# lock042/siril

Measured on AMD Instinct MI355X. Metric: Mpix/s stacked (100x6000x4000 fp32 sigma-clip) at 1/2/4/8 MI355X; % HBM roofline, higher is better.
Workload: dtype f32

## Files before the change

include/sirilgpu.h:

```cpp
#ifndef SIRILGPU_H
#define SIRILGPU_H

#include <stddef.h>
#include <stdint.h>

#ifdef __cplusplus
extern "C" {
#endif

#define SGPU_OK               0
#define SGPU_GENERIC_ERROR   (-1)
#define SGPU_SEQUENCE_ERROR  (-2)
#define SGPU_CANCEL          (-9)
#define SGPU_ALLOC_ERROR     (-10)
#define SGPU_NO_DEVICE       (-20)
#define SGPU_BAD_ARGUMENT    (-21)

enum sgpu_rejection {
	SGPU_NO_REJEC = 0, SGPU_PERCENTILE = 1, SGPU_SIGMA = 2, SGPU_MAD = 3,
	SGPU_SIGMEDIAN = 4, SGPU_WINSORIZED = 5, SGPU_LINEARFIT = 6, SGPU_GESDT = 7
};
enum sgpu_normalization {
	SGPU_NO_NORM = 0, SGPU_ADDITIVE = 1, SGPU_MULTIPLICATIVE = 2,
	SGPU_ADDITIVE_SCALING = 3, SGPU_MULTIPLICATIVE_SCALING = 4
// ... 66 lines not shown
		long *start_row, long *block_height, int *channel, int *nb_blocks, long *largest);
void sgpu_feather_mask_size(long width, long height, long *mask_width, long *mask_height);
int sgpu_feather_masks_device(sgpu_context *ctx, const void *d_frames, int elem_size, int nframes,
		long width, long height, long frame_stride, float *d_masks);
int sgpu_feather_block_area(long width, long height, long start_row, long block_height, int shifty,
		int registered, int *plane_row, int *area_h, int *mask_row, int *mask_h);
int sgpu_feather_block_device(sgpu_context *ctx, const float *d_masks, int nframes, long width,
		long height, long start_row, long block_height, const int *shifty, const int *placex,
		long canvas_width, float feather, int fits_order, float *d_planes, long plane_stride);

int sgpu_set_input_bitpix(sgpu_context *ctx, int bitpix);

long sgpu_last_exact_pixels(sgpu_context *ctx);

int sgpu_last_wz_deferred(sgpu_context *ctx, long long out[2]);

long sgpu_last_order_sensitive(sgpu_context *ctx, int *idx, long cap);

int sgpu_set_exact_only(sgpu_context *ctx, int on);


typedef struct sgpu_multi sgpu_multi;
int sgpu_multi_init(const int *devices, int ndevices, sgpu_multi **multi);
void sgpu_multi_release(sgpu_multi *multi);
int sgpu_multi_size(const sgpu_multi *multi);
sgpu_context *sgpu_multi_context(sgpu_multi *multi, int index);
int sgpu_multi_stack_rows(sgpu_multi *multi, const float *frames, int nframes, long width, long rows,
		long frame_stride, const sgpu_stack_params *params, float *out, uint16_t *rej_lo,
		uint16_t *rej_hi, uint64_t counts[2]);
int sgpu_multi_stack_rows_u16(sgpu_multi *multi, const uint16_t *frames16, int nframes, long width,
// ... 347 lines not shown
```

siril_amd/_lib.py:

```python
from __future__ import annotations

import ctypes as C
import os

PKG = os.path.dirname(os.path.abspath(__file__))
LIB_PATH = os.environ.get("SGPU_LIB") or os.path.join(PKG, "libsirilgpu.so")

EXPORTS = (
    "sgpu_abi_version", "sgpu_device_count", "sgpu_init", "sgpu_release", "sgpu_set_stream", "sgpu_synchronize",
    "sgpu_last_error", "sgpu_stack_rows", "sgpu_stack_rows_device", "sgpu_last_exact_pixels", "sgpu_last_order_sensitive",
    "sgpu_last_wz_deferred", "sgpu_set_exact_only", "sgpu_set_timing", "sgpu_last_timing", "sgpu_stack_rows_u16",
    "sgpu_stack_rows_u16_device", "sgpu_dft_shifts", "sgpu_dft_register_device",
    "sgpu_quality_estimate_device", "sgpu_quality_estimate", "sgpu_normalize_quality",
    "sgpu_quality_estimate_u16_device", "sgpu_quality_estimate_u16",
    "sgpu_fft_richardson_lucy", "sgpu_naive_richardson_lucy", "sgpu_rl_fft", "sgpu_rl_naive",
    "sgpu_rl_fft_device", "sgpu_rl_naive_device", "sgpu_rl_set_memory", "sgpu_rl_last_conv_launches",
    "sgpu_rl_last_iter_flops", "sgpu_dft_shifts_cfa", "sgpu_dft_register_cfa_device",
    "sgpu_interpolate_nongreen_device", "sgpu_debayer_buffer_new_float",
    "sgpu_debayer_buffer_superpixel_float", "sgpu_debayer_device", "sgpu_superpixel_device", "sgpu_free",
    "sgpu_debayer_buffer_new_ushort", "sgpu_debayer_u16_device",
    "sgpu_bgnoise_device", "sgpu_bgnoise_u16_device", "sgpu_bgnoise", "sgpu_bgnoise_u16",
    "sgpu_stack_seq", "sgpu_stack_seq_ex", "sgpu_norm_stats_device", "sgpu_norm_stats",
    "sgpu_norm_stats_u16_device", "sgpu_norm_stats_u16", "sgpu_norm_factors",
    "sgpu_fits_info", "sgpu_fits_read_rows", "sgpu_fits_read_rows_ex", "sgpu_fits_write",
    "sgpu_norm_to_0_1_range_device", "sgpu_multi_init", "sgpu_multi_release", "sgpu_multi_size",
    "sgpu_multi_context", "sgpu_multi_stack_rows", "sgpu_multi_stack_rows_u16", "sgpu_row_bands",
# ... 122 lines not shown
        L.sgpu_stack_rows_planes.argtypes = [vp, vp, vp, vp] + list(L.sgpu_stack_rows.argtypes[2:])
        L.sgpu_stack_rows_planes_device.restype = C.c_int
        L.sgpu_stack_rows_planes_device.argtypes = [vp, vp, vp, vp] + list(L.sgpu_stack_rows_device.argtypes[2:])
        L.sgpu_stack_rows_u16_device.restype = C.c_int
        L.sgpu_stack_rows_u16_device.argtypes = [vp, vp, C.c_int, C.c_long, C.c_long, C.c_long,
                                                 C.POINTER(StackParams), vp, vp, vp, vp, vp]
        L.sgpu_stack_rows_u16_planes_device.restype = C.c_int
        L.sgpu_stack_rows_u16_planes_device.argtypes = [vp, vp, vp, vp] + list(L.sgpu_stack_rows_u16_device.argtypes[2:])
        L.sgpu_dft_shifts.restype = C.c_int
        L.sgpu_dft_shifts.argtypes = [vp, vp, vp, C.c_int, C.c_int, vp, vp]
        L.sgpu_dft_register_device.restype = C.c_int
        L.sgpu_dft_register_device.argtypes = [vp, vp, C.c_long, vp, C.c_long, C.c_long, C.c_int,
                                               C.c_int, vp, vp]
        L.sgpu_last_exact_pixels.restype = C.c_long
        L.sgpu_last_exact_pixels.argtypes = [vp]
        L.sgpu_last_wz_deferred.restype = C.c_int
        L.sgpu_last_wz_deferred.argtypes = [vp, vp]
        L.sgpu_last_order_sensitive.restype = C.c_long
        L.sgpu_last_order_sensitive.argtypes = [vp, vp, C.c_long]
        L.sgpu_set_exact_only.restype = C.c_int
        L.sgpu_set_exact_only.argtypes = [vp, C.c_int]
        L.sgpu_set_input_bitpix.restype = C.c_int
        L.sgpu_set_input_bitpix.argtypes = [vp, C.c_int]
        L.sgpu_set_timing.restype = C.c_int
        L.sgpu_set_timing.argtypes = [vp, C.c_int]
        L.sgpu_last_timing.restype = C.c_int
        L.sgpu_last_timing.argtypes = [vp, C.POINTER(C.c_float)]
        u, i, f = C.c_uint, C.c_int, C.c_float
        for name in ("sgpu_fft_richardson_lucy", "sgpu_naive_richardson_lucy"):
            getattr(L, name).restype = i
# ... 231 lines not shown
```

siril_amd/csrc/sgpu_capi.cpp:

```cpp
#include <hip/hip_runtime.h>

#include <algorithm>
#include <cmath>
#include <cstdio>
#include <cstdlib>
#include <cstring>
#include <string>
#include <thread>
#include <vector>

#include "../../include/sirilgpu.h"
#include "sgpu_internal.h"
#include "sgpu_kparams.h"

namespace sgpu {
int launch_sorted_16(const KParams &, hipStream_t);
int launch_sorted_32(const KParams &, hipStream_t);
int launch_sorted_64(const KParams &, hipStream_t);
int launch_sorted_128(const KParams &, hipStream_t);
int launch_sorted_256(const KParams &, hipStream_t);
int launch_sorted_512(const KParams &, hipStream_t);
int launch_sorted_1024(const KParams &, hipStream_t);
int launch_sorted16_16(const KParams &, hipStream_t);
int launch_sorted16_32(const KParams &, hipStream_t);
// ... 243 lines not shown
    return n;
}

int sgpu_last_wz_deferred(sgpu_context *c, long long out[2]) {
    if (!c || !out) return fail(SGPU_BAD_ARGUMENT, "null argument");
    out[0] = out[1] = 0;
    HIP_TRY(hipStreamSynchronize(c->stream));
    if (!c->wz_cnt.p) return SGPU_OK;
    int t[2] = {0, 0};
    HIP_TRY(hipMemcpy(t, (int *)c->wz_cnt.p + sgpu::kWzDefOff, sizeof t, hipMemcpyDeviceToHost));
    out[0] = t[0];
    out[1] = t[1];
    return SGPU_OK;
}

long sgpu_last_order_sensitive(sgpu_context *c, int *idx, long cap) {
    if (!c) return fail(SGPU_BAD_ARGUMENT, "null context");
    if (hipStreamSynchronize(c->stream) != hipSuccess) return SGPU_NO_DEVICE;
    if (!c->last_mean || !c->fb2_count.p) return 0;
    int n = 0;
    if (hipMemcpy(&n, c->fb2_count.p, sizeof(int), hipMemcpyDeviceToHost) != hipSuccess) return SGPU_NO_DEVICE;
    if (idx && cap > 0 && n > 0 &&
        hipMemcpy(idx, c->fb2_list.p, (size_t)std::min<long>(cap, n) * sizeof(int), hipMemcpyDeviceToHost) !=
            hipSuccess)
        return SGPU_NO_DEVICE;
    return n;
}

}

// ... 133 lines not shown
        if (hipGetLastError() != hipSuccess) return fail(SGPU_NO_DEVICE, "count fold launch failed");
    }
    return SGPU_OK;
}

int run_launch_body(sgpu_context *c, KParams k, bool has_shift) {
    hipStream_t s = c->stream;
    const int N = k.nframes;
    int r;
    if ((r = c->fb_list.ensure(k.npix * sizeof(int))) || (r = c->fb_count.ensure(sizeof(int))))
        return r;
    k.fb_list = (int *)c->fb_list.p;
    k.fb_count = (int *)c->fb_count.p;
    HIP_TRY(hipMemsetAsync(k.fb_count, 0, sizeof(int), s));
    if (c->wz_cnt.p) HIP_TRY(hipMemsetAsync((int *)c->wz_cnt.p + 2 * sgpu::kWzMaxChunks, 0, 3 * sizeof(int), s));
    static const int wz_mode = std::getenv("SGPU_WZ") ? std::atoi(std::getenv("SGPU_WZ")) : 2;
    static const int wz_rw = std::getenv("SGPU_WZ_RW") ? std::atoi(std::getenv("SGPU_WZ_RW")) : 64;
    k.wz_mode = wz_mode;
    k.wz_rw = wz_rw;
    if (!k.frames16 && k.rtype == SGPU_NO_REJEC) {
        if ((r = c->fb2_list.ensure(k.npix * sizeof(int))) || (r = c->fb2_count.ensure(sizeof(int)))) return r;
        k.fb2_list = (int *)c->fb2_list.p;
        k.fb2_count = (int *)c->fb2_count.p;
        HIP_TRY(hipMemsetAsync(k.fb2_count, 0, sizeof(int), s));
    }
    c->last_mean = k.rtype == SGPU_NO_REJEC && !k.frames16;
    if (k.rtype == SGPU_WINSORIZED && wz_mode) {
        if ((r = c->fb2_list.ensure(k.npix * sizeof(int))) || (r = c->fb2_count.ensure(sizeof(int)))) return r;
        k.fb2_list = (int *)c->fb2_list.p;
        k.fb2_count = (int *)c->fb2_count.p;
        HIP_TRY(hipMemsetAsync(k.fb2_count, 0, sizeof(int), s));
        const int npw = sorted_capacity(N);
        const long long R = npw <= 128 ? 64 : npw / 2 + 16;
// ... 428 lines not shown
```

siril_amd/csrc/sgpu_kparams.h:

```cpp
#pragma once
#include <stdint.h>

namespace sgpu {

enum Rejection : int {
    NO_REJEC = 0, PERCENTILE = 1, SIGMA = 2, MAD = 3, SIGMEDIAN = 4,
    WINSORIZED = 5, LINEARFIT = 6, GESDT = 7,
    KMEDIAN = 16
};
enum Normalization : int {
    NO_NORM = 0, ADDITIVE = 1, MULTIPLICATIVE = 2, ADDITIVE_SCALING = 3,
    MULTIPLICATIVE_SCALING = 4
};

struct KParams {
    const float *frames;
    long long frame_stride;
    long long npix;
    int W;
    int nframes;
    int rtype;
    float sig0, sig1;
    int norm;
    const double *scale, *offset, *mul;
// ... 12 lines not shown
    int *fb_count;
    int *fb2_list;
    int *fb2_count;
    long long wz_pix0, wz_cnt;
    float *wz_ranks;
    double *wz_mom;
    int *wz_meta;
    void *wz_state;
    int *wz_list_in, *wz_list_out;
    int *wz_lcount;
    void *wz_ws;
    long long wz_ws_bytes;
    long long wz_chunk;
    int *wz_tcnt;
    int wz_mode;
    int wz_split;
    int *wz_scnt;
    int *wz_def;
    int wz_rw;
    float *scratch;
    long long scratch_threads;
    const uint16_t *frames16;
    uint16_t *out16;
    int out_f32;
    double out16_mul;
    unsigned long long *prof;
};

struct WzSplit {
    int cap;
// ... 17 lines not shown
```

siril_amd/csrc/stack_sorted_gw.h:

```cpp
#pragma once
#ifndef SGPU_GW16
#define SGPU_GW16 1, 4
#endif
#ifndef SGPU_GW16_LOOP
#define SGPU_GW16_LOOP 1, 4
#endif
#ifndef SGPU_GW32
#define SGPU_GW32 1, 4
#endif
#ifndef SGPU_GW32_LOOP
#define SGPU_GW32_LOOP 1, 4
#endif
#ifndef SGPU_GW64
#define SGPU_GW64 1, 3
#endif
#ifndef SGPU_GW64_LOOP
#define SGPU_GW64_LOOP 1, 3
#endif
#ifndef SGPU_GW128
#define SGPU_GW128 1, 2
#endif
#ifndef SGPU_GW128_LOOP
#define SGPU_GW128_LOOP 2, 4
#endif
// ... 18 lines not shown
#ifndef SGPU_WZ_PREP_G128
#define SGPU_WZ_PREP_G128 1
#endif
#ifndef SGPU_WZ_PREP_G128_XF
#define SGPU_WZ_PREP_G128_XF 1
#endif
#ifndef SGPU_WZ_PREP_W128
#define SGPU_WZ_PREP_W128 6
#endif
#ifndef SGPU_WZ_PREP_W128_G2
#define SGPU_WZ_PREP_W128_G2 4
#endif
#ifndef SGPU_WZ_PREP_W128_G1
#define SGPU_WZ_PREP_W128_G1 3
#endif
#ifndef SGPU_WZ_PREP4_RS0
#define SGPU_WZ_PREP4_RS0 20
#endif
#ifndef SGPU_WZ_PREP4_RSSTEP
#define SGPU_WZ_PREP4_RSSTEP 4
#endif
static_assert((SGPU_WZ_PREP_G128 == 1 || SGPU_WZ_PREP_G128 == 2 || SGPU_WZ_PREP_G128 == 4) &&
              (SGPU_WZ_PREP_G128_XF == 1 || SGPU_WZ_PREP_G128_XF == 2 || SGPU_WZ_PREP_G128_XF == 4),
              "prep kernel: 1, 2 or 4 lanes per pixel");
```

siril_amd/csrc/stack_sorted_inst.h:

```cpp
#pragma once
#include "stack_sorted_impl.h"
#include "stack_sorted_gw.h"
#include "stack_wz.h"
#ifndef SGPU_WZ_RRW
#define SGPU_WZ_RRW 4
#endif

#ifndef SGPU_WZ_TAIL_PASSES
#define SGPU_WZ_TAIL_PASSES 2
#endif
static_assert(SGPU_WZ_TAIL_PASSES >= 1 && SGPU_WZ_TAIL_PASSES <= 2,
              "each of the two stripe-counter sets is zeroed once per chunk and appended to by one pass");

#include <algorithm>
#include <cstdlib>
#include <type_traits>

#ifndef SGPU_WZ_MOMENTS
#define SGPU_WZ_MOMENTS 1
#endif
#ifndef SGPU_WZ_W128
#define SGPU_WZ_W128 4
#endif
#ifndef SGPU_WZ_W
// ... 27 lines not shown
        if (hipStreamCreateWithFlags(&a->s2, hipStreamNonBlocking) != hipSuccess) return -1;
        if (hipStreamCreateWithFlags(&a->s3, hipStreamNonBlocking) != hipSuccess) return -1;
        hipEvent_t *ev[6] = {&a->start, &a->prep[0], &a->prep[1], &a->rounds[0], &a->rounds[1], &a->tails};
        for (hipEvent_t *e : ev)
            if (hipEventCreateWithFlags(e, hipEventDisableTiming) != hipSuccess) return -1;
    }
    return 0;
}

using KernelFn = void (*)(KParams);
KernelFn rs_kernel_128(int kind, int xf, int rs);
KernelFn prep4_kernel_128(int xf, int rs);
int rs_pick_prep4(int N);
KernelFn prep1_kernel_128(int xf, int rs);
int rs_pick_prep1(int N);
KernelFn rs_kernel_256(int kind, int xf, int rs);
KernelFn rs_kernel_512(int kind, int xf, int rs);
template <int NP> inline KernelFn rs_kernel(int kind, int xf, int rs) {
    if constexpr (NP == 128) return rs_kernel_128(kind, xf, rs);
    else if constexpr (NP == 256) return rs_kernel_256(kind, xf, rs);
    else if constexpr (NP == 512) return rs_kernel_512(kind, xf, rs);
    else return nullptr;
}
inline bool launch_fn(KernelFn f, unsigned grid, unsigned block, hipStream_t s, const KParams &p) {
    KParams k = p;
    void *args[] = {&k};
    return hipLaunchKernel((const void *)f, dim3(grid), dim3(block), args, 0, s) == hipSuccess;
}

inline int wz_exact_block(int N) {
    const long long per = 24ll * N;
    int t = 64;
    while (t > 4 && (long long)t * per > 65536) t >>= 1;
    return (long long)t * per <= 65536 ? t : 0;
}

constexpr int kWzMinChunks = 1;
constexpr long long kWzMinChunkPix = 1LL << 19;

template <int NP, int G, int RT, int W, int U16 = 0>
static int launch_one(const KParams &p, hipStream_t s) {
    const long long threads = p.npix * (long long)G;
    const unsigned grid = (unsigned)((threads + 255) / 256);
    constexpr int E = NP / G;
    const int rs = rs_pick(E, G, p.nframes);
    const unsigned long long es = U16 ? 2ull : 4ull;
    if ((unsigned long long)(G - 1) * (unsigned long long)p.frame_stride * es +
            (unsigned long long)p.npix * es >= 0xffffffffull)
        return 1;
    constexpr bool WZM = SGPU_WZ_MOMENTS && RT == WINSORIZED && NP >= 128;
    if constexpr (WZM) if (!U16 || (p.wz_mode >= 2 && p.wz_mode <= 4 && p.wz_ws)) {
        auto two_kernel = [&](auto pg_tag) -> int {
            constexpr int PG = decltype(pg_tag)::value;
            const bool ovl = p.wz_mode == 3 || (p.wz_mode == 2 && NP <= 128);
            const int nbuf = ovl ? 2 : 1;
            constexpr int R = RankStore<NP, PG>::R;
            constexpr int PE = NP / PG;
            constexpr int PW = (NP == 128 && !U16) ? (PG == 4 ? SGPU_WZ_PREP_W128 : PG == 2 ? SGPU_WZ_PREP_W128_G2
                                                                                            : SGPU_WZ_PREP_W128_G1)
                                                   : W;
            (void)PW;
            const long long per = (long long)R * 4 + 3 * 8 + 16 + (long long)sizeof(WzState) + 8;
            const long long wsb = (p.wz_ws_bytes / nbuf) & ~4095LL;
            long long ch = std::min<long long>(p.npix, ((wsb - 4096) / per) & ~255LL);
            ch = std::min<long long>(ch, (1LL << 23) - 256);
            ch = std::min<long long>(ch, (0xffffffffLL / R) & ~255LL);
            ch = std::min<long long>(ch, ((1LL << 32) / (4LL * NP) - 256) & ~255LL);
            static const int minch = std::getenv("SGPU_WZ_MINCH") ? std::atoi(std::getenv("SGPU_WZ_MINCH")) : kWzMinChunks;
            if (ovl && minch > 1 && p.npix > (long long)minch * kWzMinChunkPix)
                ch = std::min<long long>(ch, ((p.npix + minch - 1) / minch + 255) & ~255LL);
            if (p.wz_chunk > 0) ch = std::min<long long>(ch, (p.wz_chunk + 255) & ~255LL);
            if (ch <= 0) return 1;
            WzAux *aux = nullptr;
            hipStream_t sp = s;
            if (ovl) {
                if (wz_aux(aux)) return -1;
                sp = aux->s2;
                if (hipEventRecord(aux->start, s) != hipSuccess || hipStreamWaitEvent(sp, aux->start, 0) != hipSuccess)
                    return -1;
            }
            KParams q = p;
            int *lists[2], *cnts = nullptr;
            const long long nch = (p.npix + ch - 1) / ch;
            const int et = wz_exact_block(p.nframes);
            const bool tails = !U16 && ovl && p.wz_tcnt && nch <= kWzMaxChunks && et > 0 && p.wz_rw != 100;
            auto place = [&](int b) {
                char *base = (char *)p.wz_ws + (long long)b * wsb;
                q.wz_ranks = (float *)base;
                q.wz_mom = (double *)(base + (((long long)R * 4 * ch + 255) & ~255LL));
                q.wz_meta = (int *)((char *)q.wz_mom + 3 * 8 * ch);
                q.wz_state = (void *)((char *)q.wz_meta + 16 * ch);
                lists[0] = (int *)((char *)q.wz_state + (long long)sizeof(WzState) * ch);
                lists[1] = lists[0] + ch;
                cnts = lists[1] + ch;
            };
            KernelFn prep_rs = nullptr;
            constexpr bool kOwnPrep = NP == 128 && !U16 && (PG == 4 || PG == 1);
            if constexpr (NP == 128 && !U16 && PG == 4) {
                prep_rs = prep4_kernel_128(p.shiftx ? 1 : 0, rs_pick_prep4(p.nframes));
                if (!prep_rs) return -1;
            } else if constexpr (NP == 128 && !U16 && PG == 1) {
                prep_rs = prep1_kernel_128(p.shiftx ? 1 : 0, rs_pick_prep1(p.nframes));
                if (!prep_rs) return -1;
            } else if constexpr (!U16 && PE == 64) {
                const int prs = rs_pick(PE, PG, p.nframes);
                if (prs < PE) prep_rs = rs_kernel<NP>(0, p.shiftx ? 1 : 0, prs);
            }
            int k = 0;
            for (long long p0 = 0; p0 < p.npix; p0 += ch, k++) {
                const int b = k % nbuf;
                place(b);
                q.wz_pix0 = p0;
                q.wz_cnt = std::min(ch, p.npix - p0);
                if (tails) {
                    q.fb2_list = p.fb2_list + p0;
                    q.fb2_count = p.wz_tcnt + 2 * k;
                    q.fb_list = p.fb_list + p0;
                    q.fb_count = p.wz_tcnt + 2 * k + 1;
                }
                const unsigned g1 = (unsigned)((q.wz_cnt * PG + 255) / 256), g2 = (unsigned)((q.wz_cnt + 255) / 256);
                if (ovl && k >= nbuf && hipStreamWaitEvent(sp, aux->rounds[b], 0) != hipSuccess) return -1;
                if (prep_rs) {
                    if (!launch_fn(prep_rs, g1, 256, sp, q)) return -1;
                } else if constexpr (kOwnPrep) {
                    return -1;
                } else if (p.shiftx) hipLaunchKernelGGL((k_stack_wz_prep<NP, PG, 1, PW, PE, U16>), g1, 256, 0, sp, q);
                else hipLaunchKernelGGL((k_stack_wz_prep<NP, PG, 0, PW, PE, U16>), g1, 256, 0, sp, q);
                if (ovl && (hipEventRecord(aux->prep[b], sp) != hipSuccess ||
                            hipStreamWaitEvent(s, aux->prep[b], 0) != hipSuccess))
                    return -1;
                if constexpr (U16 && NP <= 128) {
                    if (p.wz_rw == 64)
                        hipLaunchKernelGGL((k_stack_wz_rounds_lds<NP, 1, PG>), dim3((unsigned)((q.wz_cnt + 63) / 64)), 64, 0,
                                           s, q, WzSplit{});
                    else
                        hipLaunchKernelGGL((k_stack_wz_rounds<NP, 5, 1, PG>), g2, 256, 0, s, q);
                } else if constexpr (U16) {
// ... 15 lines not shown
                        case 6: hipLaunchKernelGGL((k_stack_wz_rounds<NP, 6, 0, PG>), g2, 256, 0, s, q); break;
                        case 64:
                            if constexpr (NP <= 128) {
                                const unsigned nblk = (unsigned)((q.wz_cnt + 63) / 64);
                                WzSplit sp{};
                                if (p.wz_split > 0 && p.wz_scnt) {
                                    sp.cap = p.wz_split;
                                    sp.bps = (int)((nblk + kWzStripes - 1) / kWzStripes);
                                    sp.nstripes = (int)((nblk + sp.bps - 1) / sp.bps);
                                    sp.list_out = lists[0];
                                    sp.cnt_out = p.wz_scnt;
                                    if (hipMemsetAsync(p.wz_scnt, 0, 2 * kWzStripes * kWzStripeStep * sizeof(int), s) !=
                                        hipSuccess)
                                        return -1;
                                }
                                hipLaunchKernelGGL((k_stack_wz_rounds_lds<NP, 0, PG>), dim3(nblk), 64, 0, s, q, sp);
                                for (int pass = 0; sp.cap && pass < SGPU_WZ_TAIL_PASSES; pass++) {
                                    sp.list_in = lists[pass & 1];
                                    sp.cnt_in = p.wz_scnt + (pass & 1) * kWzStripes * kWzStripeStep;
                                    sp.list_out = lists[(pass + 1) & 1];
                                    sp.cnt_out = p.wz_scnt + ((pass + 1) & 1) * kWzStripes * kWzStripeStep;
                                    sp.def = p.wz_def ? p.wz_def + pass : nullptr;
                                    hipLaunchKernelGGL((k_stack_wz_tail<NP, PG>), dim3((unsigned)sp.nstripes * 4u), 64, 0, s, q,
                                                       sp, pass == SGPU_WZ_TAIL_PASSES - 1 ? 1 : 0);
                                }
                            } else
                                hipLaunchKernelGGL((k_stack_wz_rounds<NP, 5, 0, PG>), g2, 256, 0, s, q);
                            break;
                        default: hipLaunchKernelGGL((k_stack_wz_rounds<NP, 5, 0, PG>), g2, 256, 0, s, q); break;
                    }
                }
                if (hipGetLastError() != hipSuccess) return -1;
                if (ovl && hipEventRecord(aux->rounds[b], s) != hipSuccess) return -1;
                if (tails) {
                    if (hipStreamWaitEvent(aux->s3, aux->rounds[b], 0) != hipSuccess) return -1;
                    const unsigned lg = (unsigned)std::min<long long>((q.wz_cnt * G + 255) / 256, 512);
                    if (p.shiftx) hipLaunchKernelGGL((k_stack_sorted<NP, G, RT, 1, W, U16, 1>), lg, 256, 0, aux->s3, q);
                    else hipLaunchKernelGGL((k_stack_sorted<NP, G, RT, 0, W, U16, 1>), lg, 256, 0, aux->s3, q);
                    static const bool wave = !std::getenv("SGPU_EXACT_WAVE") || std::atoi(std::getenv("SGPU_EXACT_WAVE")) != 0;
                    if (wave) {
                        const size_t lds = (size_t)5 * ((p.nframes + 1) & ~1) * sizeof(float);
                        const unsigned wb = (unsigned)std::max<long long>(1, std::min<long long>(q.wz_cnt, 1024));
                        hipLaunchKernelGGL(k_stack_exact_wave, dim3(wb), dim3(64), lds, aux->s3, q, 0);
                    } else {
                        const size_t lds = (size_t)et * 24ull * p.nframes;
                        const long long per_cu = std::max<long long>(1, (long long)((160ull << 10) / lds));
                        const long long eb = std::max<long long>(1, std::min<long long>((q.wz_cnt + et - 1) / et,
                                                                                        256 * per_cu));
// ... 110 lines not shown
```

siril_amd/csrc/stack_sorted_rs128.hip:

```cpp
#include "stack_sorted_inst.h"
#include "stack_sorted_gw.h"

namespace sgpu {
namespace {
template <int NP, int G, int W, int RS>
KernelFn prep_rs(int xf, int rs) {
    if constexpr (RS >= NP / G) {
        return nullptr;
    } else {
        if (rs == RS) return xf ? &k_stack_wz_prep<NP, G, 1, W, RS> : &k_stack_wz_prep<NP, G, 0, W, RS>;
        return prep_rs<NP, G, W, RS + 4>(xf, rs);
    }
}
template <int W, int RS, int STEP>
KernelFn prep4(int xf, int rs) {
    constexpr int R = RS < 32 ? RS : 32;
    if (rs == R || R == 32) return xf ? &k_stack_wz_prep<128, 4, 1, W, R> : &k_stack_wz_prep<128, 4, 0, W, R>;
    if constexpr (R < 32) return prep4<W, RS + STEP, STEP>(xf, rs);
    return nullptr;
}
template <int W, int RS>
KernelFn prep1(int xf, int rs) {
    if (rs == RS || RS == 128) return xf ? &k_stack_wz_prep1<128, 1, W, RS> : &k_stack_wz_prep1<128, 0, W, RS>;
    if constexpr (RS < 128) return prep1<W, RS + 8>(xf, rs);
    return nullptr;
}
template <int NP, int RT, int G, int W, int RS>
KernelFn straight_rs(int xf, int rs) {
    constexpr int E = NP / G;
    if constexpr (RS >= E) {
        return nullptr;
    } else {
        if (rs == RS)
            return xf ? &k_stack_sorted<NP, G, RT, 1, W, 0, 0, RS> : &k_stack_sorted<NP, G, RT, 0, W, 0, 0, RS>;
        return straight_rs<NP, RT, G, W, RS + (E == 64 ? 4 : 8)>(xf, rs);
    }
}
}

// ... 5 lines not shown
        case KMEDIAN: return straight_rs<128, KMEDIAN, SGPU_GW128, 72>(xf, rs);
        default: return nullptr;
    }
}

KernelFn prep4_kernel_128(int xf, int rs) { return prep4<SGPU_WZ_PREP_W128, SGPU_WZ_PREP4_RS0, SGPU_WZ_PREP4_RSSTEP>(xf, rs); }

int rs_pick_prep4(int N) {
    const int need = (N + 3) / 4;
    for (int rs = SGPU_WZ_PREP4_RS0; rs < 32; rs += SGPU_WZ_PREP4_RSSTEP)
        if (rs >= need) return rs;
    return 32;
}

KernelFn prep1_kernel_128(int xf, int rs) { return prep1<SGPU_WZ_PREP_W128_G1, 72>(xf, rs); }

int rs_pick_prep1(int N) {
    const int rs = rs_pick(128, 1, N);
    return rs < 72 ? 72 : rs;
}
}
```

siril_amd/csrc/stack_wz.h:

```cpp
#pragma once
#include "stack_sorted_impl.h"

#ifndef SGPU_WZ_KT
#define SGPU_WZ_KT 16
#endif
#ifndef SGPU_WZ_KM
#define SGPU_WZ_KM 8
#endif
#ifndef SGPU_WZ_TRACE
#define SGPU_WZ_TRACE(ev) ((void)0)
#endif

namespace sgpu {

SG_HD unsigned umul24(unsigned a, unsigned b) {
#if defined(__HIP_DEVICE_COMPILE__)
    return __umul24(a, b);
#else
    return (a & 0xffffffu) * (b & 0xffffffu);
#endif
}

SG_HD float fnext(float r) { return __builtin_bit_cast(float, __builtin_bit_cast(uint32_t, r) + 1u); }
SG_HD float fprev(float r) { return r > 0.f ? __builtin_bit_cast(float, __builtin_bit_cast(uint32_t, r) - 1u) : 0.f; }
// ... 56 lines not shown
                if (r < KT && r < kept) base[r * stride + p] = v[e];
            }
            if (e >= eh0 && e < eln) {
                if (r >= hi0 && r < kept) base[(KT + KM + r - (kept - KT)) * stride + p] = v[e];
            }
            if (e >= em0 && e <= em1) {
                if (r >= mid0 && r < mid1 && r < kept) base[(KT + r - (kept / 2 - KM / 2)) * stride + p] = v[e];
            }
        }
#if defined(__HIP_DEVICE_COMPILE__)
        __builtin_amdgcn_fence(__ATOMIC_RELEASE, "wavefront");
        __builtin_amdgcn_wave_barrier();
        __builtin_amdgcn_fence(__ATOMIC_ACQUIRE, "wavefront");
#endif
    }
#if defined(__HIP_DEVICE_COMPILE__)
    __device__ void store_buf(const float (&v)[E], int g, int kmin, int kmax) {
        mid0 = kept / 2 - KM / 2;
        hi0 = kept - KT;
        hi0 = hi0 < 0 ? 0 : hi0;
        const int eh0 = (kmin - KT) / G - 1, eln = (kmax + G - 1) / G;
        const int em0 = (kmin / 2 - KM / 2) / G - 1, em1 = (kmax / 2 + KM / 2) / G + 1;
        hi0 = hi0 > eh0 * G ? hi0 : (eh0 > 0 ? eh0 * G : 0);
        mid1 = mid0 + KM < (em1 + 1) * G ? mid0 + KM : (em1 + 1) * G;
        mid0 = mid0 > em0 * G ? mid0 : em0 * G;
        const uint32_t S4 = (uint32_t)stride * 4u;
        const uint32_t pb = (uint32_t)p * 4u;
        const auto rlo = __builtin_amdgcn_make_buffer_rsrc(base, (short)0, (int)((uint32_t)KT * S4), 0x00020000);
        const auto rmid = __builtin_amdgcn_make_buffer_rsrc(base + (long long)KT * stride, (short)0,
                                                            (int)((uint32_t)KM * S4), 0x00020000);
        const auto rhi = __builtin_amdgcn_make_buffer_rsrc(base + (long long)(KT + KM) * stride, (short)0,
                                                           (int)((uint32_t)KT * S4), 0x00020000);
        const uint32_t blo = pb + (uint32_t)g * S4;
        const uint32_t bhi = pb + (uint32_t)(g + KT - kept) * S4;
        const uint32_t bmid = pb + (uint32_t)(g - (kept / 2 - KM / 2)) * S4;
#pragma unroll
        for (int e = 0; e < E; e++) {
            const uint32_t eo = (uint32_t)(e * G) * S4;
            const uint32_t x = __builtin_bit_cast(uint32_t, v[e]);
            if (e < (KT + G - 1) / G) __builtin_amdgcn_raw_buffer_store_b32(x, rlo, (int)(blo + eo), 0, 0);
            if (e >= eh0 && e < eln) __builtin_amdgcn_raw_buffer_store_b32(x, rhi, (int)(bhi + eo), 0, 0);
            if (e >= em0 && e <= em1) __builtin_amdgcn_raw_buffer_store_b32(x, rmid, (int)(bmid + eo), 0, 0);
        }
    }
    template <int RSL>
    __device__ void store_full(const float (&v)[E]) {
        static_assert(G == 1 && RSL % 8 == 0 && RSL - 7 - KT >= KT && RSL <= E, "one lane per pixel, N >= 65");
        mid0 = kept / 2 - KM / 2;
        mid1 = mid0 + KM;
        hi0 = kept - KT;
        const uint32_t S4 = (uint32_t)stride * 4u;
        const uint32_t pb = (uint32_t)p * 4u;
        const auto rlo = __builtin_amdgcn_make_buffer_rsrc(base, (short)0, (int)((uint32_t)KT * S4), 0x00020000);
        const auto rmid = __builtin_amdgcn_make_buffer_rsrc(base + (long long)KT * stride, (short)0,
                                                            (int)((uint32_t)KM * S4), 0x00020000);
        const auto rhi = __builtin_amdgcn_make_buffer_rsrc(base + (long long)(KT + KM) * stride, (short)0,
                                                           (int)((uint32_t)KT * S4), 0x00020000);
        const uint32_t bhi = pb + (uint32_t)(KT - kept) * S4;
        const uint32_t bmid = pb - (uint32_t)mid0 * S4;
#pragma unroll
        for (int e = 0; e < KT; e++)
            __builtin_amdgcn_raw_buffer_store_b32(__builtin_bit_cast(uint32_t, v[e]), rlo, (int)(pb + (uint32_t)e * S4), 0, 0);
#pragma unroll
        for (int e = RSL / 2 - 4 - KM / 2; e < RSL / 2 + KM / 2; e++)
            __builtin_amdgcn_raw_buffer_store_b32(__builtin_bit_cast(uint32_t, v[e]), rmid, (int)(bmid + (uint32_t)e * S4), 0, 0);
#pragma unroll
        for (int e = RSL - 7 - KT; e < RSL; e++)
            __builtin_amdgcn_raw_buffer_store_b32(__builtin_bit_cast(uint32_t, v[e]), rhi, (int)(bhi + (uint32_t)e * S4), 0, 0);
    }
#endif
    SG_HD bool fetch(int r, float &x) const {
        const bool lo_ok = r < KT && r < kept, hi_ok = r >= hi0 && r < kept, mid_ok = r >= mid0 && r < mid1;
        const int slot = lo_ok ? r : hi_ok ? KT + KM + r - (kept - KT) : KT + r - (kept / 2 - KM / 2);
        const bool ok = lo_ok || hi_ok || mid_ok;
        x = (base + p)[umul24((unsigned)(ok ? slot : 0), (unsigned)stride)];
        return ok;
    }
    SG_HD bool fetch_lo(int r, float &x) const {
        const bool hit = r < KT && r < kept;
        x = (base + p)[umul24((unsigned)(hit ? r : 0), (unsigned)stride)];
        bool ok = true;
        if (__builtin_expect(!hit, 0)) ok = fetch(r, x);
        return ok;
    }
    SG_HD bool fetch_hi(int r, float &x) const {
// ... 513 lines not shown
#endif
    const int route = bad ? 2 : wz_prepare<NP, G, RSL, SGPU_WZ_GBUF != 0>(v, g, kept, kmin, p.nframes, rs, W1, W2, c0);
    if (g == 0) {
        p.wz_mom[loc] = W1;
        p.wz_mom[p.wz_cnt + loc] = W2;
        p.wz_mom[2 * p.wz_cnt + loc] = (double)c0;
        int4 m;
        m.x = route ? -1 : kept;
        m.y = rs.hi0;
        m.z = rs.mid0;
        m.w = rs.mid1;
        reinterpret_cast<int4 *>(p.wz_meta)[loc] = m;
    }
}

template <int RSL>
__device__ __forceinline__ void wz_prepare1(float (&v)[128], int kept, int N, RankStore<128, 1> &rs, double &W1,
                                            double &W2, float &c0) {
#if defined(__HIP_DEVICE_COMPILE__)
    constexpr int E = 128, K0 = RSL - 7;
    static_assert(RSL % 8 == 0 && RSL >= 72 && RSL <= E, "real-slot buckets of rs_pick(128, 1, N)");
    sort_col<E, 1, RSL>(v, 0);
    rs.kept = kept;
    const int ra = kept / 2 - ((kept & 1) ? 0 : 1), rb = kept / 2;
    const int el = (N + SGPU_STOP_GRAN - 1) & ~(SGPU_STOP_GRAN - 1);
    double s1[SGPU_NACC], s2[SGPU_NACC];
#pragma unroll
    for (int q = 0; q < SGPU_NACC; q++) s1[q] = s2[q] = 0.0;
    float sa = 0.f, sb = 0.f;
    if (__ballot(kept < K0) == 0ull) {
        rs.store_full<RSL>(v);
#pragma unroll
        for (int e = RSL / 2 - 4; e <= RSL / 2; e++) {
            sa = (e == ra) ? v[e] : sa;
            sb = (e == rb) ? v[e] : sb;
        }
        c0 = median_from(sa, sb, kept);
        const double cd = (double)c0;
#pragma unroll
        for (int e = 0; e < RSL; e++) {
            if (e == RSL - 4 && el <= RSL - 4) break;
            const float xe = (e < K0 || v[e] < f_inf()) ? v[e] : c0;
            const double y = (double)xe - cd;
            s1[e % SGPU_NACC] += y;
            s2[e % SGPU_NACC] = fma(y, y, s2[e % SGPU_NACC]);
        }
    } else {
        int kmin = kept;
#pragma unroll
        for (int lm = 32; lm >= 1; lm >>= 1) kmin = min(kmin, __shfl_xor(kmin, lm, 64));
        kmin = __builtin_amdgcn_readfirstlane(kmin);
        rs.store_buf(v, 0, kmin, N);
        const int ew0 = kmin / 2 - 1, ew1 = N / 2;
#pragma unroll
        for (int e = 0; e <= RSL / 2; e++) {
            if (e >= ew0 && e <= ew1) {
                sa = (e == ra) ? v[e] : sa;
                sb = (e == rb) ? v[e] : sb;
            }
        }
        c0 = median_from(sa, sb, kept);
        const double cd = (double)c0;
        const int elim = el < RSL ? el : RSL;
#pragma unroll
        for (int e = 0; e < RSL; e++) {
            SG_STOP4(e, elim);
            int ke = kept;
            opaque(ke);
            const float xe = e < ke ? v[e] : c0;
            const double y = (double)xe - cd;
            s1[e % SGPU_NACC] += y;
            s2[e % SGPU_NACC] = fma(y, y, s2[e % SGPU_NACC]);
        }
    }
    W1 = s1[0];
    W2 = s2[0];
#pragma unroll
    for (int q = 1; q < SGPU_NACC; q++) {
        W1 += s1[q];
        W2 += s2[q];
    }
#endif
}

template <int NP, int XF, int W, int RSL>
__global__ __launch_bounds__(256) __attribute__((amdgpu_waves_per_eu(W, 8)))
void k_stack_wz_prep1(KParams p) {
    static_assert(NP == 128, "one lane per pixel: N <= 128");
    using RS = RankStore<NP, 1>;
    const long long loc = (long long)blockIdx.x * blockDim.x + threadIdx.x;
    if (loc >= p.wz_cnt) return;
    const long long pix = p.wz_pix0 + loc;
    int kept = 0, bad = 0;
    float v[NP];
    gather_column<XF, NP, 1, true, 0, RSL, SGPU_GATHER_SLOTSTEP, true>(p, v, pix, (int)(pix % p.W), 0, kept, bad);
    opaque(bad);
    RS rs;
// ... 218 lines not shown
        } else if (route == 2) {
            const int slot = wave_append(p.fb_count, true);
            p.fb_list[slot] = (int)pix;
        } else {
            double res = o.res;
            if (is_weighted(p)) res = weighted_mean<U16>(p, pix, (int)(pix % p.W), o.pmin, o.pmax, o.nkept);
            if constexpr (U16) write_result16(p, pix, res, o.rl, o.rh);
            else write_result(p, pix, res, o.rl, o.rh);
            rl = o.rl;
            rh = o.rh;
        }
    }
    add_counts(p, rl, rh);
}

template <int NP, int PG = NP / 64>
__global__ __launch_bounds__(64) void k_stack_wz_tail(KParams p, WzSplit sp, int last) {
    using RS = RankStore<NP, 1>;
    __shared__ float s_rank[RS::R * 64];
    const int lane = (int)threadIdx.x;
    const int stripe = (int)(blockIdx.x % (unsigned)sp.nstripes);
    const int t0 = (int)(blockIdx.x / (unsigned)sp.nstripes), tstep = (int)(gridDim.x / (unsigned)sp.nstripes);
    const int seg = stripe * sp.bps * 64;
    int n = sp.cnt_in[stripe * kWzStripeStep];
    n = n < sp.bps * 64 ? n : sp.bps * 64;
    if (t0 == 0 && lane == 0 && n > 0 && sp.def) atomicAdd(sp.def, n);
    int rl = 0, rh = 0;
    for (int i0 = t0 * 64; i0 < n; i0 += tstep * 64) {
        const bool live = i0 + lane < n;
        int ent = 0;
// ... 79 lines not shown
```

siril_amd/stacking.py:

```python
from __future__ import annotations

import ctypes as C
import enum
import math
from dataclasses import dataclass, field
from typing import Optional, Sequence

import numpy as np

from ._lib import StackParams, check, lib

ST_OK, ST_GENERIC_ERROR, ST_SEQUENCE_ERROR, ST_CANCEL, ST_ALLOC_ERROR = 0, -1, -2, -9, -10


class Rejection(enum.IntEnum):
    NO_REJEC = 0
    PERCENTILE = 1
    SIGMA = 2
    MAD = 3
    SIGMEDIAN = 4
    WINSORIZED = 5
    LINEARFIT = 6
    GESDT = 7

# ... 134 lines not shown
        check(lib().sgpu_set_stream(self.h, C.c_void_p(stream_handle or 0)), "sgpu_set_stream")

    def synchronize(self):
        check(lib().sgpu_synchronize(self.h), "sgpu_synchronize")

    def set_timing(self, on: bool):
        check(lib().sgpu_set_timing(self.h, int(on)), "sgpu_set_timing")

    def last_timing(self):
        ms = (C.c_float * 2)()
        check(lib().sgpu_last_timing(self.h, ms), "sgpu_last_timing")
        return float(ms[0]), float(ms[1])

    def last_exact_pixels(self) -> int:
        return int(lib().sgpu_last_exact_pixels(self.h))

    def last_wz_deferred(self):
        a = (C.c_longlong * 2)()
        check(lib().sgpu_last_wz_deferred(self.h, a), "sgpu_last_wz_deferred")
        return int(a[0]), int(a[1])

    def set_seq_readers(self, readers: int):
        check(lib().sgpu_set_seq_readers(self.h, int(readers)), "sgpu_set_seq_readers")

    def release_seq_buffers(self):
        check(lib().sgpu_release_seq_buffers(self.h), "sgpu_release_seq_buffers")

    def last_seq_stats(self) -> dict:
        a = (C.c_double * 12)()
        check(lib().sgpu_last_seq_stats(self.h, a), "sgpu_last_seq_stats")
# ... 256 lines not shown
```

Before: 2878.

## Fuse winsorized prep and rounds kernels for N<=128 single-lane path

Adds a fused kernel for the winsorized sigma-clip path at NP=128 with one lane per pixel. It gathers, sorts, keeps the rank store in LDS and runs the finish rounds in one launch. Until now a prep kernel wrote ranks to a global workspace and a separate rounds kernel read them back. The fused kernel is used by default when sigmas are at least 3 and there is no x shift, and it skips the overlapping two-stream pipeline. Deferred pixels still spill ranks to global memory for the tail passes. The change removes a global round trip and a launch, but the large LDS footprint per block may limit occupancy. A fallback-count query API is also added.

```diff
diff --git a/include/sirilgpu.h b/include/sirilgpu.h
--- a/include/sirilgpu.h
+++ b/include/sirilgpu.h
@@ -104,6 +104,8 @@
 long sgpu_last_exact_pixels(sgpu_context *ctx);
 
 int sgpu_last_wz_deferred(sgpu_context *ctx, long long out[2]);
+
+long sgpu_last_wz_fallback(sgpu_context *ctx);
 
 long sgpu_last_order_sensitive(sgpu_context *ctx, int *idx, long cap);
 
diff --git a/siril_amd/_lib.py b/siril_amd/_lib.py
--- a/siril_amd/_lib.py
+++ b/siril_amd/_lib.py
@@ -9,7 +9,7 @@
 EXPORTS = (
     "sgpu_abi_version", "sgpu_device_count", "sgpu_init", "sgpu_release", "sgpu_set_stream", "sgpu_synchronize",
     "sgpu_last_error", "sgpu_stack_rows", "sgpu_stack_rows_device", "sgpu_last_exact_pixels", "sgpu_last_order_sensitive",
-    "sgpu_last_wz_deferred", "sgpu_set_exact_only", "sgpu_set_timing", "sgpu_last_timing", "sgpu_stack_rows_u16",
+    "sgpu_last_wz_deferred", "sgpu_last_wz_fallback", "sgpu_set_exact_only", "sgpu_set_timing", "sgpu_last_timing", "sgpu_stack_rows_u16",
     "sgpu_stack_rows_u16_device", "sgpu_dft_shifts", "sgpu_dft_register_device",
     "sgpu_quality_estimate_device", "sgpu_quality_estimate", "sgpu_normalize_quality",
     "sgpu_quality_estimate_u16_device", "sgpu_quality_estimate_u16",
@@ -162,6 +162,8 @@
                                                C.c_int, vp, vp]
         L.sgpu_last_exact_pixels.restype = C.c_long
         L.sgpu_last_exact_pixels.argtypes = [vp]
+        L.sgpu_last_wz_fallback.restype = C.c_long
+        L.sgpu_last_wz_fallback.argtypes = [vp]
         L.sgpu_last_wz_deferred.restype = C.c_int
         L.sgpu_last_wz_deferred.argtypes = [vp, vp]
         L.sgpu_last_order_sensitive.restype = C.c_long
diff --git a/siril_amd/csrc/sgpu_capi.cpp b/siril_amd/csrc/sgpu_capi.cpp
--- a/siril_amd/csrc/sgpu_capi.cpp
+++ b/siril_amd/csrc/sgpu_capi.cpp
@@ -281,6 +281,22 @@
     return SGPU_OK;
 }
 
+long sgpu_last_wz_fallback(sgpu_context *c) {
+    if (!c) return fail(SGPU_BAD_ARGUMENT, "null context");
+    if (hipStreamSynchronize(c->stream) != hipSuccess) return SGPU_NO_DEVICE;
+    if (c->last_mean || !c->fb2_count.p) return 0;
+    int n = 0;
+    if (hipMemcpy(&n, c->fb2_count.p, sizeof(int), hipMemcpyDeviceToHost) != hipSuccess) return SGPU_NO_DEVICE;
+    long total = n;
+    if (c->wz_cnt.p) {
+        std::vector<int> t(2 * sgpu::kWzMaxChunks);
+        if (hipMemcpy(t.data(), c->wz_cnt.p, t.size() * sizeof(int), hipMemcpyDeviceToHost) != hipSuccess)
+            return SGPU_NO_DEVICE;
+        for (int k = 0; k < sgpu::kWzMaxChunks; k++) total += t[2 * k];
+    }
+    return total;
+}
+
 long sgpu_last_order_sensitive(sgpu_context *c, int *idx, long cap) {
     if (!c) return fail(SGPU_BAD_ARGUMENT, "null context");
     if (hipStreamSynchronize(c->stream) != hipSuccess) return SGPU_NO_DEVICE;
@@ -444,9 +460,11 @@
     k.fb_count = (int *)c->fb_count.p;
     HIP_TRY(hipMemsetAsync(k.fb_count, 0, sizeof(int), s));
     if (c->wz_cnt.p) HIP_TRY(hipMemsetAsync((int *)c->wz_cnt.p + 2 * sgpu::kWzMaxChunks, 0, 3 * sizeof(int), s));
-    static const int wz_mode = std::getenv("SGPU_WZ") ? std::atoi(std::getenv("SGPU_WZ")) : 2;
+    static const int wz_env = std::getenv("SGPU_WZ") ? std::atoi(std::getenv("SGPU_WZ")) : -1;
+    static const int wz_mode = wz_env < 0 || wz_env == 7 ? 2 : wz_env;
     static const int wz_rw = std::getenv("SGPU_WZ_RW") ? std::atoi(std::getenv("SGPU_WZ_RW")) : 64;
     k.wz_mode = wz_mode;
+    k.wz_fused = wz_env == 7 ? 1 : (wz_env < 0 ? 2 : 0);
     k.wz_rw = wz_rw;
     if (!k.frames16 && k.rtype == SGPU_NO_REJEC) {
         if ((r = c->fb2_list.ensure(k.npix * sizeof(int))) || (r = c->fb2_count.ensure(sizeof(int)))) return r;
diff --git a/siril_amd/csrc/sgpu_kparams.h b/siril_amd/csrc/sgpu_kparams.h
--- a/siril_amd/csrc/sgpu_kparams.h
+++ b/siril_amd/csrc/sgpu_kparams.h
@@ -50,6 +50,7 @@
     long long wz_chunk;
     int *wz_tcnt;
     int wz_mode;
+    int wz_fused;
     int wz_split;
     int *wz_scnt;
     int *wz_def;
diff --git a/siril_amd/csrc/stack_sorted_gw.h b/siril_amd/csrc/stack_sorted_gw.h
--- a/siril_amd/csrc/stack_sorted_gw.h
+++ b/siril_amd/csrc/stack_sorted_gw.h
@@ -56,6 +56,9 @@
 #ifndef SGPU_WZ_PREP_W128_G1
 #define SGPU_WZ_PREP_W128_G1 3
 #endif
+#ifndef SGPU_WZ_FUSED_W128
+#define SGPU_WZ_FUSED_W128 3
+#endif
 #ifndef SGPU_WZ_PREP4_RS0
 #define SGPU_WZ_PREP4_RS0 20
 #endif
diff --git a/siril_amd/csrc/stack_sorted_inst.h b/siril_amd/csrc/stack_sorted_inst.h
--- a/siril_amd/csrc/stack_sorted_inst.h
+++ b/siril_amd/csrc/stack_sorted_inst.h
@@ -65,6 +65,8 @@
 int rs_pick_prep4(int N);
 KernelFn prep1_kernel_128(int xf, int rs);
 int rs_pick_prep1(int N);
+using FusedFn = void (*)(KParams, WzSplit);
+FusedFn fused1_kernel_128(int xf, int rs);
 KernelFn rs_kernel_256(int kind, int xf, int rs);
 KernelFn rs_kernel_512(int kind, int xf, int rs);
 template <int NP> inline KernelFn rs_kernel(int kind, int xf, int rs) {
@@ -88,6 +90,8 @@
 
 constexpr int kWzMinChunks = 1;
 constexpr long long kWzMinChunkPix = 1LL << 19;
+
+inline bool wz_fused_auto(const KParams &p) { return !p.shiftx && p.sig0 >= 3.f && p.sig1 >= 3.f; }
 
 template <int NP, int G, int RT, int W, int U16 = 0>
 static int launch_one(const KParams &p, hipStream_t s) {
@@ -103,7 +107,9 @@
     if constexpr (WZM) if (!U16 || (p.wz_mode >= 2 && p.wz_mode <= 4 && p.wz_ws)) {
         auto two_kernel = [&](auto pg_tag) -> int {
             constexpr int PG = decltype(pg_tag)::value;
-            const bool ovl = p.wz_mode == 3 || (p.wz_mode == 2 && NP <= 128);
+            const bool fused = NP == 128 && !U16 && PG == 1 && p.wz_mode == 2 && p.wz_rw == 64 &&
+                               (p.wz_fused == 1 || (p.wz_fused == 2 && wz_fused_auto(p)));
+            const bool ovl = !fused && (p.wz_mode == 3 || (p.wz_mode == 2 && NP <= 128));
             const int nbuf = ovl ? 2 : 1;
             constexpr int R = RankStore<NP, PG>::R;
             constexpr int PE = NP / PG;
@@ -124,6 +130,7 @@
             if (ch <= 0) return 1;
             WzAux *aux = nullptr;
             hipStream_t sp = s;
+            if (fused && wz_aux(aux)) return -1;
             if (ovl) {
                 if (wz_aux(aux)) return -1;
                 sp = aux->s2;
@@ -134,7 +141,7 @@
             int *lists[2], *cnts = nullptr;
             const long long nch = (p.npix + ch - 1) / ch;
             const int et = wz_exact_block(p.nframes);
-            const bool tails = !U16 && ovl && p.wz_tcnt && nch <= kWzMaxChunks && et > 0 && p.wz_rw != 100;
+            const bool tails = !U16 && (ovl || fused) && p.wz_tcnt && nch <= kWzMaxChunks && et > 0 && p.wz_rw != 100;
             auto place = [&](int b) {
                 char *base = (char *)p.wz_ws + (long long)b * wsb;
                 q.wz_ranks = (float *)base;
@@ -157,6 +164,10 @@
                 const int prs = rs_pick(PE, PG, p.nframes);
                 if (prs < PE) prep_rs = rs_kernel<NP>(0, p.shiftx ? 1 : 0, prs);
             }
+            FusedFn fused_fn = nullptr;
+            if constexpr (NP == 128 && !U16 && PG == 1) {
+                if (fused && !(fused_fn = fused1_kernel_128(p.shiftx ? 1 : 0, rs_pick_prep1(p.nframes)))) return -1;
+            }
             int k = 0;
             for (long long p0 = 0; p0 < p.npix; p0 += ch, k++) {
                 const int b = k % nbuf;
@@ -171,7 +182,8 @@
                 }
                 const unsigned g1 = (unsigned)((q.wz_cnt * PG + 255) / 256), g2 = (unsigned)((q.wz_cnt + 255) / 256);
                 if (ovl && k >= nbuf && hipStreamWaitEvent(sp, aux->rounds[b], 0) != hipSuccess) return -1;
-                if (prep_rs) {
+                if (fused) {
+                } else if (prep_rs) {
                     if (!launch_fn(prep_rs, g1, 256, sp, q)) return -1;
                 } else if constexpr (kOwnPrep) {
                     return -1;
@@ -217,7 +229,15 @@
                                         hipSuccess)
                                         return -1;
                                 }
-                                hipLaunchKernelGGL((k_stack_wz_rounds_lds<NP, 0, PG>), dim3(nblk), 64, 0, s, q, sp);
+                                if (fused) {
+                                    KParams qa = q;
+                                    WzSplit spa = sp;
+                                    void *args[] = {&qa, &spa};
+                                    if (hipLaunchKernel((const void *)fused_fn, dim3((nblk + 3) / 4), dim3(256), args, 0, s) !=
+                                        hipSuccess)
+                                        return -1;
+                                } else
+                                    hipLaunchKernelGGL((k_stack_wz_rounds_lds<NP, 0, PG>), dim3(nblk), 64, 0, s, q, sp);
                                 for (int pass = 0; sp.cap && pass < SGPU_WZ_TAIL_PASSES; pass++) {
                                     sp.list_in = lists[pass & 1];
                                     sp.cnt_in = p.wz_scnt + (pass & 1) * kWzStripes * kWzStripeStep;
@@ -234,7 +254,7 @@
                     }
                 }
                 if (hipGetLastError() != hipSuccess) return -1;
-                if (ovl && hipEventRecord(aux->rounds[b], s) != hipSuccess) return -1;
+                if ((ovl || (fused && tails)) && hipEventRecord(aux->rounds[b], s) != hipSuccess) return -1;
                 if (tails) {
                     if (hipStreamWaitEvent(aux->s3, aux->rounds[b], 0) != hipSuccess) return -1;
                     const unsigned lg = (unsigned)std::min<long long>((q.wz_cnt * G + 255) / 256, 512);
diff --git a/siril_amd/csrc/stack_sorted_rs128.hip b/siril_amd/csrc/stack_sorted_rs128.hip
--- a/siril_amd/csrc/stack_sorted_rs128.hip
+++ b/siril_amd/csrc/stack_sorted_rs128.hip
@@ -23,6 +23,12 @@
 KernelFn prep1(int xf, int rs) {
     if (rs == RS || RS == 128) return xf ? &k_stack_wz_prep1<128, 1, W, RS> : &k_stack_wz_prep1<128, 0, W, RS>;
     if constexpr (RS < 128) return prep1<W, RS + 8>(xf, rs);
+    return nullptr;
+}
+template <int W, int RS>
+FusedFn fused1(int xf, int rs) {
+    if (rs == RS || RS == 128) return xf ? &k_stack_wz_fused1<128, 1, W, RS> : &k_stack_wz_fused1<128, 0, W, RS>;
+    if constexpr (RS < 128) return fused1<W, RS + 8>(xf, rs);
     return nullptr;
 }
 template <int NP, int RT, int G, int W, int RS>
@@ -58,6 +64,7 @@
 }
 
 KernelFn prep1_kernel_128(int xf, int rs) { return prep1<SGPU_WZ_PREP_W128_G1, 72>(xf, rs); }
+FusedFn fused1_kernel_128(int xf, int rs) { return fused1<SGPU_WZ_FUSED_W128, 72>(xf, rs); }
 
 int rs_pick_prep1(int N) {
     const int rs = rs_pick(128, 1, N);
diff --git a/siril_amd/csrc/stack_wz.h b/siril_amd/csrc/stack_wz.h
--- a/siril_amd/csrc/stack_wz.h
+++ b/siril_amd/csrc/stack_wz.h
@@ -94,8 +94,10 @@
         __builtin_amdgcn_fence(__ATOMIC_ACQUIRE, "wavefront");
 #endif
     }
-#if defined(__HIP_DEVICE_COMPILE__)
-    __device__ void store_buf(const float (&v)[E], int g, int kmin, int kmax) {
+    SG_HD void drop(int region0, int size, int slot, float x) {
+        if (slot >= 0 && slot < size) base[(long long)(region0 + slot) * stride + p] = x;
+    }
+    SG_HD void store_buf(const float (&v)[E], int g, int kmin, int kmax) {
         mid0 = kept / 2 - KM / 2;
         hi0 = kept - KT;
         hi0 = hi0 < 0 ? 0 : hi0;
@@ -104,6 +106,7 @@
         hi0 = hi0 > eh0 * G ? hi0 : (eh0 > 0 ? eh0 * G : 0);
         mid1 = mid0 + KM < (em1 + 1) * G ? mid0 + KM : (em1 + 1) * G;
         mid0 = mid0 > em0 * G ? mid0 : em0 * G;
+#if defined(__HIP_DEVICE_COMPILE__)
         const uint32_t S4 = (uint32_t)stride * 4u;
         const uint32_t pb = (uint32_t)p * 4u;
         const auto rlo = __builtin_amdgcn_make_buffer_rsrc(base, (short)0, (int)((uint32_t)KT * S4), 0x00020000);
@@ -122,13 +125,22 @@
             if (e >= eh0 && e < eln) __builtin_amdgcn_raw_buffer_store_b32(x, rhi, (int)(bhi + eo), 0, 0);
             if (e >= em0 && e <= em1) __builtin_amdgcn_raw_buffer_store_b32(x, rmid, (int)(bmid + eo), 0, 0);
         }
+#else
+        for (int e = 0; e < E; e++) {
+            const int r = e * G + g;
+            if (e < (KT + G - 1) / G) drop(0, KT, r, v[e]);
+            if (e >= eh0 && e < eln) drop(KT + KM, KT, r + KT - kept, v[e]);
+            if (e >= em0 && e <= em1) drop(KT, KM, r - (kept / 2 - KM / 2), v[e]);
+        }
+#endif
     }
     template <int RSL>
-    __device__ void store_full(const float (&v)[E]) {
+    SG_HD void store_full(const float (&v)[E]) {
         static_assert(G == 1 && RSL % 8 == 0 && RSL - 7 - KT >= KT && RSL <= E, "one lane per pixel, N >= 65");
         mid0 = kept / 2 - KM / 2;
         mid1 = mid0 + KM;
         hi0 = kept - KT;
+#if defined(__HIP_DEVICE_COMPILE__)
         const uint32_t S4 = (uint32_t)stride * 4u;
         const uint32_t pb = (uint32_t)p * 4u;
         const auto rlo = __builtin_amdgcn_make_buffer_rsrc(base, (short)0, (int)((uint32_t)KT * S4), 0x00020000);
@@ -147,8 +159,37 @@
 #pragma unroll
         for (int e = RSL - 7 - KT; e < RSL; e++)
             __builtin_amdgcn_raw_buffer_store_b32(__builtin_bit_cast(uint32_t, v[e]), rhi, (int)(bhi + (uint32_t)e * S4), 0, 0);
-    }
-#endif
+#else
+        for (int e = 0; e < KT; e++) drop(0, KT, e, v[e]);
+        for (int e = RSL / 2 - 4 - KM / 2; e < RSL / 2 + KM / 2; e++) drop(KT, KM, e - mid0, v[e]);
+        for (int e = RSL - 7 - KT; e < RSL; e++) drop(KT + KM, KT, e + KT - kept, v[e]);
+#endif
+    }
+    template <int RSL>
+    SG_HD void store_full_lds(const float (&v)[E]) {
+        static_assert(G == 1 && RSL % 8 == 0 && RSL - 7 - KT >= KT && RSL <= E, "one lane per pixel, N >= 65");
+        static_assert(RSL - 7 >= KT + KM && KM / 2 <= KT && 7 <= KM, "a slot under a region stays inside the next one");
+        mid0 = kept / 2 - KM / 2;
+        mid1 = mid0 + KM;
+        hi0 = kept - KT;
+        const int S = (int)stride;
+        float *const bl = base + p;
+        float *const bh = bl + (KT + KM - hi0) * S;
+        float *const bm = bl + (KT - mid0) * S;
+#pragma unroll
+        for (int e = RSL - 7 - KT; e < RSL; e++)
+            if (e < RSL - 7 || e < kept) bh[e * S] = v[e];
+#pragma unroll
+        for (int e = RSL / 2 - 4 - KM / 2; e < RSL / 2 + KM / 2; e++)
+            if (e < RSL / 2 || e < mid1) bm[e * S] = v[e];
+#pragma unroll
+        for (int e = 0; e < KT; e++) bl[e * S] = v[e];
+#if defined(__HIP_DEVICE_COMPILE__)
+        __builtin_amdgcn_fence(__ATOMIC_RELEASE, "wavefront");
+        __builtin_amdgcn_wave_barrier();
+        __builtin_amdgcn_fence(__ATOMIC_ACQUIRE, "wavefront");
+#endif
+    }
     SG_HD bool fetch(int r, float &x) const {
         const bool lo_ok = r < KT && r < kept, hi_ok = r >= hi0 && r < kept, mid_ok = r >= mid0 && r < mid1;
         const int slot = lo_ok ? r : hi_ok ? KT + KM + r - (kept - KT) : KT + r - (kept / 2 - KM / 2);
@@ -692,13 +733,26 @@
     }
 }
 
-template <int RSL>
-__device__ __forceinline__ void wz_prepare1(float (&v)[128], int kept, int N, RankStore<128, 1> &rs, double &W1,
-                                            double &W2, float &c0) {
+SG_HD bool wave_any(bool x) {
 #if defined(__HIP_DEVICE_COMPILE__)
+    return __ballot(x) != 0ull;
+#else
+    return x;
+#endif
+}
+SG_HD int wave_min(int x) {
+#if defined(__HIP_DEVICE_COMPILE__)
+#pragma unroll
+    for (int lm = 32; lm >= 1; lm >>= 1) x = min(x, __shfl_xor(x, lm, 64));
+    x = __builtin_amdgcn_readfirstlane(x);
+#endif
+    return x;
+}
+template <int RSL, bool LDS = false>
+SG_HD void wz_prepare1_sorted(const float (&v)[128], int kept, int N, RankStore<128, 1> &rs, double &W1, double &W2,
+                              float &c0) {
     constexpr int E = 128, K0 = RSL - 7;
     static_assert(RSL % 8 == 0 && RSL >= 72 && RSL <= E, "real-slot buckets of rs_pick(128, 1, N)");
-    sort_col<E, 1, RSL>(v, 0);
     rs.kept = kept;
     const int ra = kept / 2 - ((kept & 1) ? 0 : 1), rb = kept / 2;
     const int el = (N + SGPU_STOP_GRAN - 1) & ~(SGPU_STOP_GRAN - 1);
@@ -706,8 +760,9 @@
 #pragma unroll
     for (int q = 0; q < SGPU_NACC; q++) s1[q] = s2[q] = 0.0;
     float sa = 0.f, sb = 0.f;
-    if (__ballot(kept < K0) == 0ull) {
-        rs.store_full<RSL>(v);
+    if (!wave_any(kept < K0)) {
+        if constexpr (LDS) rs.template store_full_lds<RSL>(v);
+        else rs.template store_full<RSL>(v);
 #pragma unroll
         for (int e = RSL / 2 - 4; e <= RSL / 2; e++) {
             sa = (e == ra) ? v[e] : sa;
@@ -724,11 +779,9 @@
             s2[e % SGPU_NACC] = fma(y, y, s2[e % SGPU_NACC]);
         }
     } else {
-        int kmin = kept;
-#pragma unroll
-        for (int lm = 32; lm >= 1; lm >>= 1) kmin = min(kmin, __shfl_xor(kmin, lm, 64));
-        kmin = __builtin_amdgcn_readfirstlane(kmin);
-        rs.store_buf(v, 0, kmin, N);
+        const int kmin = wave_min(kept);
+        if constexpr (LDS) rs.store(v, 0, kmin, N);
+        else rs.store_buf(v, 0, kmin, N);
         const int ew0 = kmin / 2 - 1, ew1 = N / 2;
 #pragma unroll
         for (int e = 0; e <= RSL / 2; e++) {
@@ -758,7 +811,12 @@
         W1 += s1[q];
         W2 += s2[q];
     }
-#endif
+}
+
+template <int RSL, bool LDS = false>
+SG_HD void wz_prepare1(float (&v)[128], int kept, int N, RankStore<128, 1> &rs, double &W1, double &W2, float &c0) {
+    sort_col<128, 1, RSL>(v, 0);
+    wz_prepare1_sorted<RSL, LDS>(v, kept, N, rs, W1, W2, c0);
 }
 
 template <int NP, int XF, int W, int RSL>
@@ -1007,6 +1065,91 @@
     add_counts(p, rl, rh);
 }
 
+template <int NP, int XF, int W, int RSL>
+__global__ __launch_bounds__(256) __attribute__((amdgpu_waves_per_eu(W, 8)))
+void k_stack_wz_fused1(KParams p, WzSplit sp) {
+    static_assert(NP == 128, "one lane per pixel: N <= 128");
+    using RS = RankStore<NP, 1>;
+    __shared__ float s_rank[4 * RS::R * 64];
+    if (((long long)blockIdx.x * 4 + (threadIdx.x >> 6)) * 64 >= p.wz_cnt) return;
+    int kept = 0, bad = 0;
+    double W1, W2;
+    float c0;
+    RS rs;
+    float v[NP];
+    {
+        const long long c = ((long long)blockIdx.x * 4 + (threadIdx.x >> 6)) * 64, l = c + (threadIdx.x & 63);
+        const long long gp = p.wz_pix0 + (l < p.wz_cnt ? l : c);
+        gather_column<XF, NP, 1, true, 0, RSL, SGPU_GATHER_SLOTSTEP, true>(p, v, gp, (int)(gp % p.W), 0, kept, bad);
+    }
+    opaque(bad);
+    sort_col<NP, 1, RSL>(v, 0);
+    int tid = (int)threadIdx.x;
+    opaque(tid);
+    const int lane = tid & 63;
+    const long long tile = (long long)blockIdx.x * 4 + (tid >> 6);
+    const long long col0 = tile * 64;
+    const long long loc = col0 + lane;
+    const bool live = loc < p.wz_cnt;
+    const long long pix = p.wz_pix0 + (live ? loc : col0);
+    float *const tile_rank = s_rank + (tid >> 6) * (RS::R * 64);
+    rs.base = tile_rank;
+    rs.stride = 64;
+    rs.p = lane;
+    wz_prepare1_sorted<RSL, true>(v, kept, p.nframes, rs, W1, W2, c0);
+    int rl = 0, rh = 0;
+    if (live) {
+        int route = 2;
+        PixOut o;
+        WzState st;
+        if (!bad && kept > 0) {
+            const int N = p.nframes;
+            const int el = (N + SGPU_STOP_GRAN - 1) & ~(SGPU_STOP_GRAN - 1);
+            route = wz_finish_cap<0>(rs, kept, W1, W2, c0, el, p.sig0, p.sig1, sp.cap, o, st);
+        }
+        if (route == kWzDeferred) {
+            const unsigned long long dm = __ballot(true);
+            const int ci = (int)__popcll(dm & ((1ull << lane) - 1ull));
+            const int tw = (int)(p.wz_cnt - col0 < 64 ? p.wz_cnt - col0 : 64);
+            const int stripe = (int)tile / sp.bps;
+            const int slot = wave_append(sp.cnt_out + stripe * kWzStripeStep, true);
+            sp.list_out[stripe * sp.bps * 64 + slot] = wz_entry((int)tile, ci, lane);
+            reinterpret_cast<WzState *>(p.wz_state)[loc] = st;
+            p.wz_mom[loc] = W1;
+            p.wz_mom[p.wz_cnt + loc] = W2;
+            p.wz_mom[2 * p.wz_cnt + loc] = (double)c0;
+            reinterpret_cast<int4 *>(p.wz_meta)[loc] = make_int4(kept, rs.hi0, rs.mid0, rs.mid1);
+            if (tw == 64 && (p.wz_cnt & 3) == 0) {
+                const unsigned cnt = (unsigned)p.wz_cnt, c0w = (unsigned)col0;
+#pragma unroll 2
+                for (int j = 0; j < RS::R; j += 4) {
+                    const unsigned f = (unsigned)(ci * RS::R + j);
+                    const float4 q = make_float4(tile_rank[j * 64 + lane], tile_rank[(j + 1) * 64 + lane],
+                                                 tile_rank[(j + 2) * 64 + lane], tile_rank[(j + 3) * 64 + lane]);
+                    *reinterpret_cast<float4 *>(p.wz_ranks + (umul24(f >> 6, cnt) + c0w + (f & 63u))) = q;
+                }
+            } else {
+#pragma unroll 4
+                for (int j = 0; j < RS::R; j++)
+                    p.wz_ranks[wz_crec_index(ci * RS::R + j, tw, p.wz_cnt, col0)] = tile_rank[j * 64 + lane];
+            }
+        } else if (route == 1) {
+            const int slot = wave_append(p.fb2_count, true);
+            p.fb2_list[slot] = (int)pix;
+        } else if (route == 2) {
+            const int slot = wave_append(p.fb_count, true);
+            p.fb_list[slot] = (int)pix;
+        } else {
+            double res = o.res;
+            if (is_weighted(p)) res = weighted_mean<0>(p, pix, (int)(pix % p.W), o.pmin, o.pmax, o.nkept);
+            write_result(p, pix, res, o.rl, o.rh);
+            rl = o.rl;
+            rh = o.rh;
+        }
+    }
+    add_counts(p, rl, rh);
+}
+
 template <int NP, int PG = NP / 64>
 __global__ __launch_bounds__(64) void k_stack_wz_tail(KParams p, WzSplit sp, int last) {
     using RS = RankStore<NP, 1>;
diff --git a/siril_amd/stacking.py b/siril_amd/stacking.py
--- a/siril_amd/stacking.py
+++ b/siril_amd/stacking.py
@@ -172,6 +172,9 @@
 
     def last_exact_pixels(self) -> int:
         return int(lib().sgpu_last_exact_pixels(self.h))
+
+    def last_wz_fallback(self) -> int:
+        return int(lib().sgpu_last_wz_fallback(self.h))
 
     def last_wz_deferred(self):
         a = (C.c_longlong * 2)()
```

Result: faster. 3081, median of 6 (+7.1%).
